# Equim-chan/Mortal

Hardware: NVIDIA H100
Metric: table-steps/sec batched self-play (higher is better)
Workload: dtype u8/i32 env + bf16 policy net

## Files before the change

include/mjx.h:

```cpp
#ifndef MJX_H
#define MJX_H
#include <stdint.h>

#ifdef __cplusplus
extern "C" {
#endif

enum mjx_status { MJX_OK = 0, MJX_ERR_CUDA = -1, MJX_ERR_ARG = -2, MJX_ERR_TABLES = -3, MJX_ERR_STATE = -4 };

#define MJX_ACTION_SPACE 46
#define MJX_OBS_COLS 34
#define MJX_MAX_ROWS_PER_TABLE 3

typedef struct mjx_env mjx_env;

const char* mjx_last_error(void);

int mjx_init(const char* data_dir, int device);

int mjx_obs_rows(int version);

int mjx_env_create(mjx_env** out, int n_tables, const uint64_t* nonces_host, const uint64_t* keys_host,
                   int obs_version, int shuffle_kind, int enable_quick_eval);
void mjx_env_destroy(mjx_env* env);
// ... 141 lines not shown
        forbidden_tiles[34], discarded_tiles[34];
    uint8_t akas_seen[3], akas_in_hand[3];
    uint8_t bakaze, jikaze, kyoku, honba, kyotaku, rank, oya, is_all_last;
    int32_t scores[4];
    uint8_t n_dora_indicators, dora_indicators[5];
    uint8_t riichi_declared[4], riichi_accepted[4];
    uint8_t at_turn, tiles_left;
    int8_t shanten, real_time_shanten;
    uint8_t has_last_self_tsumo, last_self_tsumo, has_last_kawa_tile, last_kawa_tile;
    uint32_t cans;
    uint8_t n_ankan_candidates, ankan_candidates[3], n_kakan_candidates, kakan_candidates[3];
    uint8_t chankan_chance, can_w_riichi, is_w_riichi, at_rinshan, at_ippatsu, at_furiten, to_mark_same_cycle_furiten,
        kans_on_board, is_menzen;
    uint8_t n_chis, chis[4], n_pons, pons[4], n_minkans, minkans[4], n_ankans, ankans[4];
    uint8_t doras_owned[4], doras_seen, tehai_len_div3, has_next_shanten_discard;
    uint8_t kawa_len[4];
    uint8_t viewer, pad_[3];
    int32_t err;
} mjx_player_view;
int mjx_state_create(mjx_env** out, int n, const uint8_t* player_ids_host, int obs_version);
int mjx_state_update(mjx_env* env, const uint64_t* words_host, const uint64_t* payload_host, uint32_t* cans_host);
int mjx_state_view(mjx_env* env, int index, mjx_player_view* out_host);
int mjx_state_rows(mjx_env* env, const uint8_t* at_kan_select_host, void* stream);
int mjx_state_query(mjx_env* env, int index, int what, const int32_t* args, int32_t* out);
int mjx_state_copy(mjx_env* dst, int dst_index, mjx_env* src, int src_index);

int mjx_env_set_encode_timing(mjx_env* env, int enable);
int mjx_env_last_encode_ms(mjx_env* env, float* ms_features, float* ms_store);

long long mjx_env_launch_count(mjx_env* env);

int mjx_env_row_cap(mjx_env* env);
uint8_t* mjx_env_masks(mjx_env* env);
int32_t* mjx_env_row_table(mjx_env* env);
uint8_t* mjx_env_row_seat(mjx_env* env);
uint32_t* mjx_env_row_step(mjx_env* env);
int32_t* mjx_env_num_rows_dev(mjx_env* env);

int mjx_env_results(mjx_env* env, void* stream, int32_t* scores_host , uint8_t* ranks_host ,
                    int32_t* steps_host , int32_t* err_host , int32_t* done_host );

int mjx_env_policy_test(mjx_env* env, int kind, int64_t* actions_dev, int64_t* trace_dev, float* q_values_dev,
                        void* stream);

int mjx_nn_affine_mish_bf16(const void* x, const float* scale, const float* bias, void* out, long long n_elems, int channels,
                            void* stream);
int mjx_nn_pool_bf16(const void* x, void* avg, void* mx, int batch, int length, int channels, void* stream);
int mjx_nn_gate_residual_bf16(const void* y, const void* gate, const void* x, void* out, int batch, int length, int channels,
                              void* stream);
int mjx_nn_obs_to_nhwc_bf16(const float* obs, void* out, int batch, int channels, int length, int channels_padded, void* stream);
int mjx_nn_block_tail_bf16(const void* y, const void* x, const float* w1, const float* b1, const float* w2t, const float* b2,
                           const float* scale, const float* bias, void* gate_scratch , void* x_out,
                           void* a_out, int batch, int length, int channels, int hidden, void* stream);

int mjx_shanten(const uint8_t* tiles_dev, const uint8_t* len_div3_dev, int8_t* out_dev, int n, void* stream);

typedef struct mjx_agari_in {
    uint8_t tehai[34];
    uint8_t chis[4], pons[4], minkans[4], ankans[4];
    uint8_t n_chis, n_pons, n_minkans, n_ankans;
    uint8_t bakaze, jikaze, winning_tile, is_ron;
    uint8_t additional_hans, doras;
    uint8_t is_oya, pad;
} mjx_agari_in;
typedef struct mjx_agari_out {
    uint8_t kind;
    uint8_t fu, han, yakuman;
    int32_t ron, tsumo_ko, tsumo_oya;
} mjx_agari_out;
int mjx_agari(const mjx_agari_in* in_dev, mjx_agari_out* out_dev, int n, int mode, void* stream);

int mjx_shanten_host(const uint8_t* tiles, const uint8_t* len_div3, int8_t* out, int n);
int mjx_agari_host(const mjx_agari_in* in, mjx_agari_out* out, int n, int mode);

int mjx_make_wall_host(uint64_t nonce, uint64_t key, int kyoku, int honba, int shuffle_kind, uint8_t* wall136);

#ifdef __cplusplus
}
#endif
#endif
```

mortal_b200/_lib.py:

```python
from __future__ import annotations

import ctypes as C
import os

HERE = os.path.dirname(os.path.abspath(__file__))
DATA_DIR = os.path.join(HERE, "data")
_LIB = None
_INIT_DEVICE = None


class MjxError(RuntimeError):
    pass


def lib_path() -> str:
    return os.path.join(HERE, "libmjx.so")


class AgariIn(C.Structure):
    _fields_ = [
        ("tehai", C.c_uint8 * 34),
        ("chis", C.c_uint8 * 4), ("pons", C.c_uint8 * 4), ("minkans", C.c_uint8 * 4), ("ankans", C.c_uint8 * 4),
        ("n_chis", C.c_uint8), ("n_pons", C.c_uint8), ("n_minkans", C.c_uint8), ("n_ankans", C.c_uint8),
        ("bakaze", C.c_uint8), ("jikaze", C.c_uint8), ("winning_tile", C.c_uint8), ("is_ron", C.c_uint8),
        ("additional_hans", C.c_uint8), ("doras", C.c_uint8), ("is_oya", C.c_uint8), ("pad", C.c_uint8),
    ]


class AgariOut(C.Structure):
    _fields_ = [("kind", C.c_uint8), ("fu", C.c_uint8), ("han", C.c_uint8), ("yakuman", C.c_uint8),
                ("ron", C.c_int32), ("tsumo_ko", C.c_int32), ("tsumo_oya", C.c_int32)]


SYMBOLS = {
    "mjx_last_error": (C.c_char_p, []),
    "mjx_init": (C.c_int, [C.c_char_p, C.c_int]),
    "mjx_obs_rows": (C.c_int, [C.c_int]),
    "mjx_env_create": (C.c_int, [C.POINTER(C.c_void_p), C.c_int, C.c_void_p, C.c_void_p, C.c_int, C.c_int, C.c_int]),
    "mjx_env_destroy": (None, [C.c_void_p]),
    "mjx_env_step": (C.c_int, [C.c_void_p, C.c_void_p, C.c_void_p, C.c_void_p]),
    "mjx_env_set_quick_eval": (C.c_int, [C.c_void_p, C.c_void_p]),
    "mjx_env_set_agari_guard": (C.c_int, [C.c_void_p, C.c_void_p]),
    "mjx_env_encode_obs": (C.c_int, [C.c_void_p, C.c_void_p, C.c_void_p]),
    "mjx_oracle_obs_rows": (C.c_int, [C.c_int]),
    "mjx_env_encode_invisible": (C.c_int, [C.c_void_p, C.c_void_p, C.c_int, C.c_void_p]),
    "mjx_env_set_obs_version": (C.c_int, [C.c_void_p, C.c_int]),
    "mjx_state_create": (C.c_int, [C.POINTER(C.c_void_p), C.c_int, C.c_void_p, C.c_int]),
    "mjx_state_update": (C.c_int, [C.c_void_p, C.c_void_p, C.c_void_p, C.c_void_p]),
    "mjx_state_view": (C.c_int, [C.c_void_p, C.c_int, C.c_void_p]),
    "mjx_state_rows": (C.c_int, [C.c_void_p, C.c_void_p, C.c_void_p]),
    "mjx_state_query": (C.c_int, [C.c_void_p, C.c_int, C.c_int, C.c_void_p, C.c_void_p]),
    "mjx_state_copy": (C.c_int, [C.c_void_p, C.c_int, C.c_void_p, C.c_int]),
    "mjx_env_set_sp": (C.c_int, [C.c_void_p, C.c_int]),
    "mjx_env_encode_obs_host": (C.c_int, [C.c_void_p, C.c_void_p, C.c_void_p, C.c_void_p, C.POINTER(C.c_int), C.c_void_p]),
    "mjx_env_encode_obs_host_begin": (C.c_int, [C.c_void_p, C.c_void_p, C.c_void_p, C.c_void_p, C.POINTER(C.c_int), C.c_void_p]),
    "mjx_env_encode_obs_host_finish": (C.c_int, [C.c_void_p]),
    "mjx_env_sp_overflows": (C.c_int, [C.c_void_p, C.c_void_p, C.POINTER(C.c_int)]),
    "mjx_env_sp_stats": (C.c_int, [C.c_void_p, C.c_void_p, C.POINTER(C.c_int)]),
    "mjx_env_enable_grp": (C.c_int, [C.c_void_p, C.c_int]),
    "mjx_env_read_grp": (C.c_int, [C.c_void_p, C.c_void_p, C.c_void_p, C.c_void_p]),
    "mjx_env_enable_log": (C.c_int, [C.c_void_p, C.c_int]),
    "mjx_env_log_len_dev": (C.c_void_p, [C.c_void_p]),
    "mjx_env_read_log": (C.c_int, [C.c_void_p, C.c_void_p, C.c_void_p, C.c_void_p]),
    "mjx_env_log_words_dev": (C.c_void_p, [C.c_void_p]),
    "mjx_meta_record_dev": (C.c_int, [C.c_longlong] + [C.c_void_p] * 4 + [C.c_int, C.c_int] + [C.c_void_p] * 5 + [C.c_int, C.c_int]
                            + [C.c_void_p] * 7 + [C.c_longlong, C.c_longlong, C.c_void_p]),
    "mjx_mjai_render_count_dev": (C.c_int, [C.c_int, C.c_void_p, C.c_void_p, C.c_int, C.c_void_p, C.c_int, C.c_int, C.c_void_p,
                                            C.c_void_p, C.c_void_p, C.c_void_p, C.c_void_p, C.c_longlong, C.c_void_p, C.c_void_p,
                                            C.c_void_p]),
    "mjx_mjai_render_fill_dev": (C.c_int, [C.c_int, C.c_void_p, C.c_void_p, C.c_int, C.c_void_p, C.c_int, C.c_int, C.c_void_p,
                                           C.c_void_p, C.c_void_p, C.c_void_p, C.c_void_p, C.c_longlong, C.c_void_p, C.c_void_p,
                                           C.c_int, C.c_int, C.c_void_p, C.c_longlong, C.c_void_p]),
    "mjx_nn_affine_mish_bf16": (C.c_int, [C.c_void_p, C.c_void_p, C.c_void_p, C.c_void_p, C.c_longlong, C.c_int, C.c_void_p]),
    "mjx_nn_pool_bf16": (C.c_int, [C.c_void_p, C.c_void_p, C.c_void_p, C.c_int, C.c_int, C.c_int, C.c_void_p]),
    "mjx_nn_gate_residual_bf16": (C.c_int, [C.c_void_p, C.c_void_p, C.c_void_p, C.c_void_p, C.c_int, C.c_int, C.c_int, C.c_void_p]),
    "mjx_nn_obs_to_nhwc_bf16": (C.c_int, [C.c_void_p, C.c_void_p, C.c_int, C.c_int, C.c_int, C.c_int, C.c_void_p]),
    "mjx_nn_block_tail_bf16": (C.c_int, [C.c_void_p] * 11 + [C.c_int, C.c_int, C.c_int, C.c_int, C.c_void_p]),
    "mjx_env_create_replay": (C.c_int, [C.POINTER(C.c_void_p), C.c_int, C.c_void_p, C.c_void_p, C.c_void_p, C.c_longlong, C.c_void_p,
                                        C.c_void_p, C.c_longlong, C.c_void_p, C.c_int, C.c_int]),
    "mjx_env_create_replay_dev": (C.c_int, [C.POINTER(C.c_void_p), C.c_int, C.c_void_p, C.c_void_p, C.c_void_p, C.c_longlong,
                                            C.c_void_p, C.c_void_p, C.c_longlong, C.c_void_p, C.c_int, C.c_int, C.c_void_p]),
    "mjx_env_replay_trust_seeds": (C.c_int, [C.c_void_p, C.c_void_p, C.c_void_p, C.c_int]),
    "mjx_env_replay_step": (C.c_int, [C.c_void_p, C.c_void_p]),
    "mjx_env_replay_viewpoints": (C.c_int, [C.c_void_p, C.c_void_p]),
    "mjx_env_row_label": (C.c_void_p, [C.c_void_p]),
    "mjx_env_row_meta": (C.c_void_p, [C.c_void_p]),
    "mjx_env_set_encode_timing": (C.c_int, [C.c_void_p, C.c_int]),
    "mjx_env_last_encode_ms": (C.c_int, [C.c_void_p, C.POINTER(C.c_float), C.POINTER(C.c_float)]),
    "mjx_env_launch_count": (C.c_longlong, [C.c_void_p]),
    "mjx_env_num_rows": (C.c_int, [C.c_void_p, C.c_void_p, C.POINTER(C.c_int)]),
    "mjx_env_poll": (C.c_int, [C.c_void_p, C.c_void_p, C.POINTER(C.c_int)]),
    "mjx_env_num_live": (C.c_int, [C.c_void_p, C.c_void_p, C.POINTER(C.c_int)]),
    "mjx_env_total_steps": (C.c_int, [C.c_void_p, C.c_void_p, C.POINTER(C.c_int64)]),
    "mjx_env_row_cap": (C.c_int, [C.c_void_p]),
    "mjx_env_masks": (C.c_void_p, [C.c_void_p]),
    "mjx_env_row_table": (C.c_void_p, [C.c_void_p]),
    "mjx_env_row_seat": (C.c_void_p, [C.c_void_p]),
    "mjx_env_row_step": (C.c_void_p, [C.c_void_p]),
    "mjx_env_num_rows_dev": (C.c_void_p, [C.c_void_p]),
    "mjx_env_results": (C.c_int, [C.c_void_p, C.c_void_p, C.c_void_p, C.c_void_p, C.c_void_p, C.c_void_p, C.c_void_p]),
    "mjx_env_policy_test": (C.c_int, [C.c_void_p, C.c_int, C.c_void_p, C.c_void_p, C.c_void_p, C.c_void_p]),
    "mjx_shanten": (C.c_int, [C.c_void_p, C.c_void_p, C.c_void_p, C.c_int, C.c_void_p]),
    "mjx_agari": (C.c_int, [C.c_void_p, C.c_void_p, C.c_int, C.c_int, C.c_void_p]),
    "mjx_shanten_host": (C.c_int, [C.c_void_p, C.c_void_p, C.c_void_p, C.c_int]),
    "mjx_agari_host": (C.c_int, [C.c_void_p, C.c_void_p, C.c_int, C.c_int]),
    "mjx_make_wall_host": (C.c_int, [C.c_uint64, C.c_uint64, C.c_int, C.c_int, C.c_int, C.c_void_p]),
    "mjx_validate_logs": (C.c_int, [C.c_int, C.c_void_p, C.c_void_p, C.c_void_p, C.c_longlong, C.c_void_p, C.c_void_p, C.c_longlong,
                                    C.c_void_p, C.c_void_p, C.c_longlong, C.c_void_p, C.c_void_p]),
    "mjx_validate_logs_dev": (C.c_int, [C.c_int, C.c_void_p, C.c_void_p, C.c_void_p, C.c_longlong, C.c_void_p, C.c_void_p,
                                        C.c_longlong, C.c_void_p, C.c_void_p, C.c_longlong, C.c_void_p, C.c_void_p]),
    "mjx_mjai_count_dev": (C.c_int, [C.c_int, C.c_void_p, C.c_longlong, C.c_void_p, C.c_int, C.c_void_p, C.c_void_p]),
    "mjx_mjai_fill_dev": (C.c_int, [C.c_int, C.c_void_p, C.c_longlong, C.c_void_p, C.c_int, C.c_void_p, C.c_void_p, C.c_void_p,
                                    C.c_void_p, C.c_void_p, C.c_void_p, C.c_longlong, C.c_void_p, C.c_longlong, C.c_void_p,
                                    C.c_longlong, C.c_void_p]),
    "mjx_mjai_fill_deltas_dev": (C.c_int, [C.c_int, C.c_void_p, C.c_longlong, C.c_void_p, C.c_int, C.c_void_p, C.c_void_p,
                                           C.c_void_p, C.c_void_p, C.c_void_p, C.c_void_p, C.c_longlong, C.c_void_p, C.c_longlong,
                                           C.c_void_p, C.c_longlong, C.c_void_p, C.c_void_p, C.c_void_p]),
    "mjx_stat_logs_dev": (C.c_int, [C.c_int, C.c_void_p, C.c_void_p, C.c_void_p, C.c_longlong, C.c_void_p, C.c_void_p, C.c_longlong,
                                    C.c_void_p, C.c_void_p, C.c_void_p, C.c_void_p, C.c_void_p, C.c_void_p]),
    "mjx_grp_logs_dev": (C.c_int, [C.c_int, C.c_void_p, C.c_void_p, C.c_void_p, C.c_longlong, C.c_void_p, C.c_void_p, C.c_longlong,
                                   C.c_void_p, C.c_void_p, C.c_void_p, C.c_void_p, C.c_void_p, C.c_void_p, C.c_void_p]),
}


def load():
    global _LIB
    if _LIB is not None:
        return _LIB
    path = lib_path()
    if not os.path.exists(path):
# ... 25 lines not shown
```

mortal_b200/csrc/mjx_kernels.cu:

```cuda
#include <cstdio>
#include <cstring>
#include <mutex>
#include <string>
#include <vector>

#include "../../include/mjx.h"
#include "mjx_sp.cuh"
#include "mjx_policy.cuh"
#include "mjx_replay.cuh"
#include "mjx_validate.cuh"
#include "mjx_mjai.cuh"
#include "mjx_mjai_write.cuh"
#include "mjx_stat.cuh"
#include "mjx_grp.cuh"
#include "mjx_invisible.cuh"
#include "mjx_state.cuh"
#include "mjx_nn.cuh"
#include "mjx_tables_host.h"

using namespace mjx;

constexpr int STEP_WARPS = 4;

__global__ void __launch_bounds__(STEP_WARPS * 32) k_step(EnvView V, Tables T) {
    __shared__ __align__(16) unsigned char s_tab[STEP_WARPS][sizeof(TableState)];
    __shared__ WarpScratch s_scratch[STEP_WARPS];
    const int warp = threadIdx.x >> 5, lane = threadIdx.x & 31;
    const int table = blockIdx.x * STEP_WARPS + warp;
    if (table >= V.n_tables) return;
    TableState* g = V.tables + table;
    if (!(g->gflags & GF_ALIVE)) return;
    constexpr int NV = sizeof(TableState) / 16;
    uint4* dst = reinterpret_cast<uint4*>(s_tab[warp]);
    const uint4* src = reinterpret_cast<const uint4*>(g);
    for (int i = lane; i < NV; i += 32) dst[i] = src[i];
    __syncwarp();
    Ctx c;
    c.S = reinterpret_cast<TableState*>(s_tab[warp]);
    c.W = &s_scratch[warp];
    c.T = T;
    c.lane = lane;
    c.df = s_scratch[warp].dora_factor;
    if (V.log) { c.log = V.log + (size_t)table * V.log_cap; c.log_n = V.log_len + table; c.log_cap = V.log_cap; }
    if (V.grp) { c.grp = V.grp + (size_t)table * V.grp_cap * 7; c.grp_n = V.grp_len + table; c.grp_cap = V.grp_cap; }
    const i32 err_before = c.S->err;
    const bool live = step_table(c, V, table);
    __syncwarp();
    uint4* gdst = reinterpret_cast<uint4*>(g);
    for (int i = lane; i < NV; i += 32) gdst[i] = dst[i];
    if (lane == 0 && live) {
        atomicAdd(&V.counters[0], 1ull);
        atomicAdd(&V.counters[1], 1ull);
    }
    if (lane == 0 && err_before == 0 && c.S->err != 0) atomicAdd(&V.counters[2], 1ull);
}

__global__ void __launch_bounds__(STEP_WARPS * 32) k_replay_step(EnvView V, ReplayView R, Tables T) {
    __shared__ __align__(16) unsigned char s_tab[STEP_WARPS][sizeof(TableState)];
    __shared__ WarpScratch s_scratch[STEP_WARPS];
    const int warp = threadIdx.x >> 5, lane = threadIdx.x & 31;
    const int job = blockIdx.x * STEP_WARPS + warp;
    if (job >= V.n_tables) return;
    TableState* g = V.tables + job;
    if (!(g->gflags & GF_ALIVE)) return;
    constexpr int NV = sizeof(TableState) / 16;
    uint4* dst = reinterpret_cast<uint4*>(s_tab[warp]);
    const uint4* src = reinterpret_cast<const uint4*>(g);
    for (int i = lane; i < NV; i += 32) dst[i] = src[i];
    __syncwarp();
    Ctx c;
// ... 1741 lines not shown
int mjx_nn_affine_mish_bf16(const void* x, const float* scale, const float* bias, void* out, long long n_elems, int channels,
                            void* stream) {
    if (!x || !scale || !bias || !out || channels <= 0 || channels % 8 || n_elems % channels)
        return fail(MJX_ERR_ARG, "mjx_nn_affine_mish_bf16: bad arguments");
    if (!g_ready) return fail(MJX_ERR_STATE, "mjx_nn_*: call mjx_init first");
    const size_t n_vec = (size_t)n_elems / 8;
    mjx_nn::k_affine_mish<<<nn_grid_for(n_vec, channels / 8), 256, 0, (cudaStream_t)stream>>>((const mjx_nn::Vec8*)x, scale, bias, (mjx_nn::Vec8*)out,
                                                                            n_vec, channels / 8);
    CU(cudaGetLastError());
    return MJX_OK;
}
int mjx_nn_pool_bf16(const void* x, void* avg, void* mx, int batch, int length, int channels, void* stream) {
    if (!x || !avg || !mx || batch <= 0 || length <= 0 || channels <= 0 || channels % 8)
        return fail(MJX_ERR_ARG, "mjx_nn_pool_bf16: bad arguments");
    if (!g_ready) return fail(MJX_ERR_STATE, "mjx_nn_*: call mjx_init first");
    mjx_nn::k_pool<<<nn_grid((size_t)batch * (channels / 8)), 256, 0, (cudaStream_t)stream>>>(
        (const mjx_nn::Vec8*)x, (mjx_nn::Vec8*)avg, (mjx_nn::Vec8*)mx, batch, length, channels / 8);
    CU(cudaGetLastError());
    return MJX_OK;
}
int mjx_nn_obs_to_nhwc_bf16(const float* obs, void* out, int batch, int channels, int length, int channels_padded, void* stream) {
    if (!obs || !out || batch <= 0 || channels <= 0 || length <= 0 || length > 128 || channels_padded < channels ||
        channels_padded % mjx_nn::NHWC_TC)
        return fail(MJX_ERR_ARG, "mjx_nn_obs_to_nhwc_bf16: bad arguments (channels_padded a multiple of 64, length <= 128)");
    if (!g_ready) return fail(MJX_ERR_STATE, "mjx_nn_*: call mjx_init first");
    const size_t smem = (size_t)mjx_nn::NHWC_TC * (length + 1) * sizeof(float);
    const long long grid = (long long)batch * (channels_padded / mjx_nn::NHWC_TC);
    if (grid > 0x7fffffffLL) return fail(MJX_ERR_ARG, "mjx_nn_obs_to_nhwc_bf16: batch too large");
    mjx_nn::k_obs_to_nhwc<<<(int)grid, 256, smem, (cudaStream_t)stream>>>(obs, (__nv_bfloat16*)out, channels, length, channels_padded);
    CU(cudaGetLastError());
    return MJX_OK;
}
int mjx_nn_block_tail_bf16(const void* y, const void* x, const float* w1, const float* b1, const float* w2t, const float* b2,
                           const float* scale, const float* bias, void* gate_scratch, void* x_out, void* a_out, int batch, int length,
                           int channels, int hidden, void* stream) {
    if (!y || !x || !w1 || !b1 || !w2t || !b2 || !scale || !bias || !gate_scratch || !x_out || !a_out || batch <= 0 || length <= 0 ||
        channels <= 0 || channels % 8 || channels > 256 || hidden <= 0 || hidden > 64)
        return fail(MJX_ERR_ARG, "mjx_nn_block_tail_bf16: bad arguments (channels % 8 == 0, <= 256; hidden <= 64)");
    if (!g_ready) return fail(MJX_ERR_STATE, "mjx_nn_*: call mjx_init first");
    cudaStream_t st = (cudaStream_t)stream;
    const int c8 = channels / 8;
    const int warps_per_cta = 8;
    const int grid = std::max(1, std::min((batch + warps_per_cta - 1) / warps_per_cta, g_sm_count * 8));
    mjx_nn::k_pool_gate<<<grid, warps_per_cta * 32, 0, st>>>((const mjx_nn::Vec8*)y, w1, b1, w2t, b2, (mjx_nn::Vec8*)gate_scratch, batch, length,
                                                               c8, hidden);
    CU(cudaGetLastError());
    const size_t n_vec = (size_t)batch * length * c8;
    mjx_nn::k_gate_residual_mish<<<nn_grid_for(n_vec, c8), 256, 0, st>>>(
        (const mjx_nn::Vec8*)y, (const mjx_nn::Vec8*)gate_scratch, (const mjx_nn::Vec8*)x, scale, bias, (mjx_nn::Vec8*)x_out,
        (mjx_nn::Vec8*)a_out, n_vec, length, c8);
    CU(cudaGetLastError());
    return MJX_OK;
}
int mjx_nn_gate_residual_bf16(const void* y, const void* gate, const void* x, void* out, int batch, int length, int channels,
                              void* stream) {
    if (!y || !gate || !x || !out || batch <= 0 || length <= 0 || channels <= 0 || channels % 8)
        return fail(MJX_ERR_ARG, "mjx_nn_gate_residual_bf16: bad arguments");
    if (!g_ready) return fail(MJX_ERR_STATE, "mjx_nn_*: call mjx_init first");
    const size_t n_vec = (size_t)batch * length * (channels / 8);
    mjx_nn::k_gate_residual<<<nn_grid(n_vec), 256, 0, (cudaStream_t)stream>>>((const mjx_nn::Vec8*)y, (const mjx_nn::Vec8*)gate,
                                                                              (const mjx_nn::Vec8*)x, (mjx_nn::Vec8*)out, n_vec,
                                                                              length, channels / 8);
    CU(cudaGetLastError());
    return MJX_OK;
}

int mjx_shanten(const uint8_t* tiles_dev, const uint8_t* len_dev, int8_t* out_dev, int n, void* stream) {
    if (!g_ready) return fail(MJX_ERR_STATE, "mjx_shanten: call mjx_init first");
    if (n <= 0) return MJX_OK;
    k_shanten<<<(n + SH_THREADS - 1) / SH_THREADS, SH_THREADS, 0, (cudaStream_t)stream>>>(g_T, tiles_dev, len_dev,
                                                                                         (i8*)out_dev, n);
    CU(cudaGetLastError());
    return MJX_OK;
}

int mjx_agari(const mjx_agari_in* in_dev, mjx_agari_out* out_dev, int n, int mode, void* stream) {
    if (!g_ready) return fail(MJX_ERR_STATE, "mjx_agari: call mjx_init first");
    if (mode < 0 || mode > 3) return fail(MJX_ERR_ARG, "mjx_agari: mode must be 0..3");
    if (n <= 0) return MJX_OK;
    k_agari<<<(n + 127) / 128, 128, 0, (cudaStream_t)stream>>>(g_T, in_dev, out_dev, n, mode);
    CU(cudaGetLastError());
    return MJX_OK;
}

namespace {
struct HostScratch {
    std::mutex mu;
    void* p[3] = {nullptr, nullptr, nullptr};
    size_t cap[3] = {0, 0, 0};
    int reserve(int i, size_t bytes, void** out) {
        if (cap[i] < bytes) {
            cudaFree(p[i]); p[i] = nullptr; cap[i] = 0;
            size_t want = 1 << 16;
            while (want < bytes) want <<= 1;
            cudaError_t e = cudaMalloc(&p[i], want);
            if (e != cudaSuccess) return fail(MJX_ERR_CUDA, cudaGetErrorString(e));
            cap[i] = want;
        }
        *out = p[i];
        return MJX_OK;
    }
};
HostScratch g_host_scratch;
}

int mjx_shanten_host(const uint8_t* tiles, const uint8_t* len_div3, int8_t* out, int n) {
// ... 48 lines not shown
```

mortal_b200/model.py:

```python
from __future__ import annotations

import torch
from torch import nn

OBS_ROWS = {1: 938, 2: 942, 3: 934, 4: 1012}
ACTION_SPACE = 46


class ChannelGate(nn.Module):
    def __init__(self, channels: int, ratio: int = 16):
        super().__init__()
        self.fc1 = nn.Linear(channels, channels // ratio)
        self.fc2 = nn.Linear(channels // ratio, channels)
        nn.init.zeros_(self.fc1.bias)
        nn.init.zeros_(self.fc2.bias)
        self.act = nn.Mish(inplace=True)

    def _mlp(self, v):
        return self.fc2(self.act(self.fc1(v)))

    def forward(self, x):
        gate = torch.sigmoid(self._mlp(x.mean(-1)) + self._mlp(x.amax(-1)))
        return x * gate.unsqueeze(-1)

# ... 24 lines not shown
        return scale.view(1, -1, 1, 1).contiguous(), shift.view(1, -1, 1, 1).contiguous()

    def forward_fast(self, x, aff, w1, w2, aff32=None):
        (s1, b1), (s2, b2) = aff
        F = torch.nn.functional
        if aff32 is not None and x.is_cuda and x.dtype == torch.bfloat16:
            from . import nn_ops

            (f1, g1), (f2, g2) = aff32
            y = F.conv2d(nn_ops.affine_mish(x, f1, g1), w1, padding=(0, 1))
            y = F.conv2d(nn_ops.affine_mish(y, f2, g2), w2, padding=(0, 1))
            avg, mx = nn_ops.pool_mean_max(y)
            h = self.gate._mlp(torch.cat((avg, mx), 0))
            gate = torch.sigmoid(h[: avg.shape[0]] + h[avg.shape[0]:])
            return nn_ops.gate_residual(y, gate.contiguous(), x)
        y = F.conv2d(F.mish(torch.addcmul(b1, x, s1)), w1, padding=(0, 1))
        y = F.conv2d(F.mish(torch.addcmul(b2, y, s2)), w2, padding=(0, 1))
        return self.gate.forward_fast(y) + x


class Brain(nn.Module):
    def __init__(self, *, conv_channels: int = 192, num_blocks: int = 40, version: int = 4):
        super().__init__()
        assert version == 4, "only the version-4 network is restated here"
        self.version = version
        c = conv_channels
        self.stem = nn.Conv1d(OBS_ROWS[version], c, 3, padding=1, bias=False)
        self.blocks = nn.Sequential(*[PreActBlock(c) for _ in range(num_blocks)])
        self.bn = nn.BatchNorm1d(c, momentum=0.01, eps=1e-3)
        self.act = nn.Mish(inplace=True)
        self.neck = nn.Conv1d(c, 32, 3, padding=1)
        self.fc = nn.Linear(32 * 34, 1024)

    def forward(self, obs):
        x = self.blocks(self.stem(obs))
        x = self.act(self.neck(self.act(self.bn(x))))
        return self.act(self.fc(x.flatten(1)))

    @torch.no_grad()
    def prepare_fast(self, dtype=None):
        assert not self.training, "prepare_fast() is for eval mode"
        flat = lambda a: (a[0].float().flatten().contiguous(), a[1].float().flatten().contiguous())
        self._aff32 = [(flat(PreActBlock._affine(b.bn1)), flat(PreActBlock._affine(b.bn2))) for b in self.blocks]
        self._aff32_out = flat(PreActBlock._affine(self.bn))
        if dtype is not None:
            self.to(dtype)
        self._aff = [(PreActBlock._affine(b.bn1), PreActBlock._affine(b.bn2)) for b in self.blocks]
        self._aff_out = PreActBlock._affine(self.bn)
        f32 = lambda t: t.detach().float().contiguous()
        self._gate32 = [(f32(b.gate.fc1.weight), f32(b.gate.fc1.bias), f32(b.gate.fc2.weight.t()), f32(b.gate.fc2.bias)) for b in self.blocks]
        cl = lambda conv: conv.weight.unsqueeze(2).contiguous(memory_format=torch.channels_last)
        self._w = [(cl(b.conv1), cl(b.conv2)) for b in self.blocks]
        self._w_stem, self._w_neck = cl(self.stem), cl(self.neck)
        cin = self.stem.weight.shape[1]
        self._cpad = (cin + 63) // 64 * 64
        wp = torch.zeros((self.stem.weight.shape[0], self._cpad, 3), dtype=self.stem.weight.dtype, device=self.stem.weight.device)
        wp[:, :cin] = self.stem.weight.detach()
        self._w_stem_pad = wp.unsqueeze(2).contiguous(memory_format=torch.channels_last)
        self._fast_dtype = dtype
        return self

    def forward_fast(self, obs):
        F = torch.nn.functional
        fused = obs.is_cuda and self._fast_dtype == torch.bfloat16
        if fused and obs.dtype == torch.float32 and obs.is_contiguous():
            from . import nn_ops

            x = F.conv2d(nn_ops.obs_to_nhwc(obs, self._cpad), self._w_stem_pad, padding=(0, 1))
        else:
            if self._fast_dtype is not None:
                obs = obs.to(self._fast_dtype)
            x = obs.unsqueeze(2).contiguous(memory_format=torch.channels_last)
            x = F.conv2d(x, self._w_stem, padding=(0, 1))
        if fused:
            from . import nn_ops

            n = len(self.blocks)
            a = nn_ops.affine_mish(x, *self._aff32[0][0]) if n else nn_ops.affine_mish(x, *self._aff32_out)
            for i in range(n):
                (w1, w2), (_, (f2, g2)) = self._w[i], self._aff32[i]
                y = F.conv2d(a, w1, padding=(0, 1))
                y = F.conv2d(nn_ops.affine_mish(y, f2, g2), w2, padding=(0, 1))
                nxt = self._aff32[i + 1][0] if i + 1 < n else self._aff32_out
                x, a = nn_ops.block_tail(y, x, *self._gate32[i], *nxt)
            x = a
        else:
            for blk, aff, (w1, w2) in zip(self.blocks, self._aff, self._w):
                x = blk.forward_fast(x, aff, w1, w2, None)
            s, b = self._aff_out
            x = F.mish(torch.addcmul(b, x, s))
        x = F.mish(F.conv2d(x, self._w_neck, self.neck.bias, padding=(0, 1)))
        return F.mish(self.fc(x.flatten(1)))


class DQN(nn.Module):
    def __init__(self, *, version: int = 4):
        super().__init__()
        assert version == 4
        self.net = nn.Linear(1024, 1 + ACTION_SPACE)
        nn.init.zeros_(self.net.bias)

    def forward(self, phi, mask):
        v, a = self.net(phi).split((1, ACTION_SPACE), dim=-1)
        a_mean = a.masked_fill(~mask, 0.0).sum(-1, keepdim=True) / mask.sum(-1, keepdim=True)
        return (v + a - a_mean).masked_fill(~mask, -torch.inf)
```

mortal_b200/nn_ops.py:

```python
from __future__ import annotations

import ctypes as C

import torch

from . import _lib


def _stream(t: torch.Tensor):
    return C.c_void_p(torch.cuda.current_stream(t.device).cuda_stream)


def _check_nhwc(x: torch.Tensor):
    assert x.is_cuda and x.dtype == torch.bfloat16 and x.dim() == 4 and x.shape[2] == 1
    b, c, _, l = x.shape
    assert c % 8 == 0 and x.stride(1) == 1 and x.stride(3) == c and x.stride(0) == c * l, "expected channels_last [B, C, 1, L]"
    return b, c, l


def affine_mish(x: torch.Tensor, scale: torch.Tensor, bias: torch.Tensor) -> torch.Tensor:
    b, c, l = _check_nhwc(x)
    assert scale.dtype == torch.float32 and bias.dtype == torch.float32 and scale.numel() == c == bias.numel()
    out = torch.empty_like(x)
    _lib.check(_lib.load().mjx_nn_affine_mish_bf16(C.c_void_p(x.data_ptr()), C.c_void_p(scale.data_ptr()), C.c_void_p(bias.data_ptr()),
                                                   C.c_void_p(out.data_ptr()), x.numel(), c, _stream(x)), "mjx_nn_affine_mish_bf16")
    return out


def pool_mean_max(x: torch.Tensor):
    b, c, l = _check_nhwc(x)
    avg = torch.empty((b, c), dtype=torch.bfloat16, device=x.device)
    mx = torch.empty((b, c), dtype=torch.bfloat16, device=x.device)
    _lib.check(_lib.load().mjx_nn_pool_bf16(C.c_void_p(x.data_ptr()), C.c_void_p(avg.data_ptr()), C.c_void_p(mx.data_ptr()), b, l, c,
                                            _stream(x)), "mjx_nn_pool_bf16")
    return avg, mx


def gate_residual(y: torch.Tensor, gate: torch.Tensor, x: torch.Tensor) -> torch.Tensor:
    b, c, l = _check_nhwc(y)
    assert _check_nhwc(x) == (b, c, l) and gate.dtype == torch.bfloat16 and gate.shape == (b, c) and gate.is_contiguous()
    out = torch.empty_like(y)
    _lib.check(_lib.load().mjx_nn_gate_residual_bf16(C.c_void_p(y.data_ptr()), C.c_void_p(gate.data_ptr()), C.c_void_p(x.data_ptr()),
                                                     C.c_void_p(out.data_ptr()), b, l, c, _stream(y)), "mjx_nn_gate_residual_bf16")
    return out


def block_tail(y: torch.Tensor, x: torch.Tensor, w1: torch.Tensor, b1: torch.Tensor, w2t: torch.Tensor, b2: torch.Tensor,
               scale: torch.Tensor, bias: torch.Tensor):
    b, c, l = _check_nhwc(y)
    assert _check_nhwc(x) == (b, c, l)
    h = w1.shape[0]
    for t, shape in ((w1, (h, c)), (b1, (h,)), (w2t, (h, c)), (b2, (c,)), (scale, (c,)), (bias, (c,))):
        assert t.dtype == torch.float32 and tuple(t.shape) == shape and t.is_contiguous() and t.is_cuda
    assert c <= 256, "block_tail: at most 256 channels"
    x_out, a_out = torch.empty_like(y), torch.empty_like(y)
    gate = torch.empty((b, c), dtype=torch.bfloat16, device=y.device)
    p = lambda t: C.c_void_p(t.data_ptr())
    _lib.check(_lib.load().mjx_nn_block_tail_bf16(p(y), p(x), p(w1), p(b1), p(w2t), p(b2), p(scale), p(bias), p(gate), p(x_out), p(a_out),
                                                  b, l, c, h, _stream(y)), "mjx_nn_block_tail_bf16")
    return x_out, a_out


def obs_to_nhwc(obs: torch.Tensor, channels_padded: int) -> torch.Tensor:
    assert obs.is_cuda and obs.dtype == torch.float32 and obs.dim() == 3 and obs.is_contiguous()
    b, c, l = obs.shape
    assert channels_padded >= c and channels_padded % 64 == 0
    out = torch.empty((b, channels_padded, 1, l), dtype=torch.bfloat16, device=obs.device, memory_format=torch.channels_last)
    _lib.check(_lib.load().mjx_nn_obs_to_nhwc_bf16(C.c_void_p(obs.data_ptr()), C.c_void_p(out.data_ptr()), b, c, l, channels_padded,
                                                   _stream(obs)), "mjx_nn_obs_to_nhwc_bf16")
    return out
```

Baseline: 245,800.

## Add warp-specialized TMA+WGMMA conv3 kernel with fused affine-mish epilogue for residual blocks

Replaces the cuDNN F.conv2d calls in each residual block with a custom Hopper kernel. It uses TMA bulk loads into an 8-stage mbarrier pipeline, a producer warpgroup, and consumer warpgroups issuing m64n192k16 WGMMA as an implicit GEMM over three taps, with boundary rows zeroed in shared memory. The first conv fuses the affine+mish epilogue, which removes a separate elementwise kernel and its memory round trip. The kernel is hardcoded to 192 channels and length 34, and the zeroing of padded rows plus the swizzle descriptors carry correctness risk.

```diff
diff --git a/include/mjx.h b/include/mjx.h
--- a/include/mjx.h
+++ b/include/mjx.h
@@ -217,6 +217,8 @@
 int mjx_nn_block_tail_bf16(const void* y, const void* x, const float* w1, const float* b1, const float* w2t, const float* b2,
                            const float* scale, const float* bias, void* gate_scratch , void* x_out,
                            void* a_out, int batch, int length, int channels, int hidden, void* stream);
+int mjx_nn_conv3_bf16(const void* x, const void* w, const float* scale, const float* bias, void* out, int batch, int length, int channels,
+                      int epilogue, void* stream);
 
 int mjx_shanten(const uint8_t* tiles_dev, const uint8_t* len_div3_dev, int8_t* out_dev, int n, void* stream);
 
diff --git a/mortal_b200/_lib.py b/mortal_b200/_lib.py
--- a/mortal_b200/_lib.py
+++ b/mortal_b200/_lib.py
@@ -76,6 +76,7 @@
     "mjx_nn_gate_residual_bf16": (C.c_int, [C.c_void_p, C.c_void_p, C.c_void_p, C.c_void_p, C.c_int, C.c_int, C.c_int, C.c_void_p]),
     "mjx_nn_obs_to_nhwc_bf16": (C.c_int, [C.c_void_p, C.c_void_p, C.c_int, C.c_int, C.c_int, C.c_int, C.c_void_p]),
     "mjx_nn_block_tail_bf16": (C.c_int, [C.c_void_p] * 11 + [C.c_int, C.c_int, C.c_int, C.c_int, C.c_void_p]),
+    "mjx_nn_conv3_bf16": (C.c_int, [C.c_void_p] * 5 + [C.c_int, C.c_int, C.c_int, C.c_int, C.c_void_p]),
     "mjx_env_create_replay": (C.c_int, [C.POINTER(C.c_void_p), C.c_int, C.c_void_p, C.c_void_p, C.c_void_p, C.c_longlong, C.c_void_p,
                                         C.c_void_p, C.c_longlong, C.c_void_p, C.c_int, C.c_int]),
     "mjx_env_create_replay_dev": (C.c_int, [C.POINTER(C.c_void_p), C.c_int, C.c_void_p, C.c_void_p, C.c_void_p, C.c_longlong,
diff --git a/mortal_b200/csrc/mjx_conv.cuh b/mortal_b200/csrc/mjx_conv.cuh
--- /dev/null
+++ b/mortal_b200/csrc/mjx_conv.cuh
@@ -0,0 +1,173 @@
+#pragma once
+#include <cuda.h>
+#include <cuda_bf16.h>
+#include <cuda_runtime.h>
+#include <stdint.h>
+
+#include "mjx_nn.cuh"
+
+namespace mjx_nn {
+
+constexpr int CV_C = 192, CV_L = 34;
+constexpr int CV_BM = 192, CV_BK = 32;
+constexpr int CV_KSTEPS = 3 * (CV_C / CV_BK);
+constexpr int CV_STAGES = 8;
+constexpr int CV_CONSUMERS = CV_BM / 64;
+constexpr int CV_THREADS = (CV_CONSUMERS + 1) * 128;
+constexpr int CV_A_BYTES = CV_BM * CV_BK * 2, CV_B_BYTES = CV_C * CV_BK * 2;
+constexpr int CV_OUT_BYTES = 64 * 64 * 2;
+constexpr int CV_SMEM = CV_STAGES * (CV_A_BYTES + CV_B_BYTES) + CV_CONSUMERS * CV_OUT_BYTES + 2 * CV_STAGES * 8 + 1024;
+enum { CV_EPI_PLAIN = 0, CV_EPI_AFFINE_MISH = 1 };
+
+__device__ __forceinline__ uint32_t cv_smem(const void* p) { return (uint32_t)__cvta_generic_to_shared(p); }
+__device__ __forceinline__ void cv_bar_init(uint32_t bar, uint32_t count) {
+    asm volatile("mbarrier.init.shared::cta.b64 [%0], %1;" ::"r"(bar), "r"(count) : "memory");
+}
+__device__ __forceinline__ void cv_bar_expect_tx(uint32_t bar, uint32_t bytes) {
+    asm volatile("mbarrier.arrive.expect_tx.shared::cta.b64 _, [%0], %1;" ::"r"(bar), "r"(bytes) : "memory");
+}
+__device__ __forceinline__ void cv_bar_arrive(uint32_t bar) {
+    asm volatile("mbarrier.arrive.shared::cta.b64 _, [%0];" ::"r"(bar) : "memory");
+}
+__device__ __forceinline__ void cv_bar_wait(uint32_t bar, uint32_t parity) {
+    uint32_t done;
+    do {
+        asm volatile("{ .reg .pred p; mbarrier.try_wait.parity.shared::cta.b64 p, [%1], %2; selp.u32 %0, 1, 0, p; }"
+                     : "=r"(done) : "r"(bar), "r"(parity) : "memory");
+    } while (!done);
+}
+__device__ __forceinline__ void cv_tma_load(uint32_t dst, const CUtensorMap* map, int c0, int c1, uint32_t bar) {
+    asm volatile("cp.async.bulk.tensor.2d.shared::cluster.global.mbarrier::complete_tx::bytes [%0], [%1, {%2, %3}], [%4];"
+                 ::"r"(dst), "l"(reinterpret_cast<uint64_t>(map)), "r"(c0), "r"(c1), "r"(bar) : "memory");
+}
+__device__ __forceinline__ void cv_tma_store(const CUtensorMap* map, int c0, int c1, uint32_t src) {
+    asm volatile("cp.async.bulk.tensor.2d.global.shared::cta.bulk_group [%0, {%1, %2}], [%3];"
+                 ::"l"(reinterpret_cast<uint64_t>(map)), "r"(c0), "r"(c1), "r"(src) : "memory");
+}
+__device__ __forceinline__ void cv_fence_async_smem() { asm volatile("fence.proxy.async.shared::cta;" ::: "memory"); }
+__device__ __forceinline__ void cv_wg_sync(int wg) {
+    asm volatile("bar.sync %0, 128;" ::"r"(wg + 1) : "memory");
+}
+
+__device__ __forceinline__ uint64_t cv_desc(uint32_t saddr) {
+    return (uint64_t)((saddr & 0x3FFFF) >> 4) | (uint64_t)1 << 16 | (uint64_t)(512 >> 4) << 32 | (uint64_t)2 << 62;
+}
+
+#define CV_D8(i) "+f"(d[i + 0]), "+f"(d[i + 1]), "+f"(d[i + 2]), "+f"(d[i + 3]), "+f"(d[i + 4]), "+f"(d[i + 5]), "+f"(d[i + 6]), "+f"(d[i + 7])
+__device__ __forceinline__ void cv_wgmma(float* d, uint64_t da, uint64_t db, int scale_d) {
+    asm volatile(
+        "{ .reg .pred p; setp.ne.b32 p, %98, 0;\n"
+        "wgmma.mma_async.sync.aligned.m64n192k16.f32.bf16.bf16 "
+        "{%0, %1, %2, %3, %4, %5, %6, %7, %8, %9, %10, %11, %12, %13, %14, %15, %16, %17, %18, %19, %20, %21, %22, %23, "
+        "%24, %25, %26, %27, %28, %29, %30, %31, %32, %33, %34, %35, %36, %37, %38, %39, %40, %41, %42, %43, %44, %45, %46, %47, "
+        "%48, %49, %50, %51, %52, %53, %54, %55, %56, %57, %58, %59, %60, %61, %62, %63, %64, %65, %66, %67, %68, %69, %70, %71, "
+        "%72, %73, %74, %75, %76, %77, %78, %79, %80, %81, %82, %83, %84, %85, %86, %87, %88, %89, %90, %91, %92, %93, %94, %95}, "
+        "%96, %97, p, 1, 1, 0, 0; }\n"
+        : CV_D8(0), CV_D8(8), CV_D8(16), CV_D8(24), CV_D8(32), CV_D8(40), CV_D8(48), CV_D8(56), CV_D8(64), CV_D8(72), CV_D8(80), CV_D8(88)
+        : "l"(da), "l"(db), "r"(scale_d));
+}
+#undef CV_D8
+
+template <int EPI>
+__global__ void __launch_bounds__(CV_THREADS, 1) k_conv3_wgmma(const __grid_constant__ CUtensorMap map_a, const __grid_constant__ CUtensorMap map_w,
+                                                               const __grid_constant__ CUtensorMap map_out, const float* __restrict__ scale,
+                                                               const float* __restrict__ bias, int m_rows) {
+    extern __shared__ uint8_t cv_raw[];
+    const uint32_t base = (cv_smem(cv_raw) + 1023) & ~1023u;
+    uint8_t* const gbase = cv_raw + (base - cv_smem(cv_raw));
+    const uint32_t sa = base, sb = sa + CV_STAGES * CV_A_BYTES, so = sb + CV_STAGES * CV_B_BYTES;
+    const uint32_t full = so + CV_CONSUMERS * CV_OUT_BYTES, empty = full + CV_STAGES * 8;
+    const int n_tiles = (m_rows + CV_BM - 1) / CV_BM;
+    const int tid = threadIdx.x, wg = tid >> 7;
+
+    if (tid == 0) {
+        for (int s = 0; s < CV_STAGES; s++) {
+            cv_bar_init(full + 8 * s, 1);
+            cv_bar_init(empty + 8 * s, CV_CONSUMERS);
+        }
+        asm volatile("fence.mbarrier_init.release.cluster;" ::: "memory");
+        cv_fence_async_smem();
+    }
+    __syncthreads();
+
+    if (wg == CV_CONSUMERS) {
+        asm volatile("setmaxnreg.dec.sync.aligned.u32 40;");
+        if (tid == CV_CONSUMERS * 128) {
+            int it = 0;
+            for (int tile = blockIdx.x; tile < n_tiles; tile += gridDim.x) {
+                for (int ks = 0; ks < CV_KSTEPS; ks++, it++) {
+                    const int s = it % CV_STAGES, tap = ks % 3, c0 = (ks / 3) * CV_BK;
+                    cv_bar_wait(empty + 8 * s, ((it / CV_STAGES) & 1) ^ 1);
+                    cv_bar_expect_tx(full + 8 * s, CV_A_BYTES + CV_B_BYTES);
+                    cv_tma_load(sa + s * CV_A_BYTES, &map_a, c0, tile * CV_BM + tap - 1, full + 8 * s);
+                    cv_tma_load(sb + s * CV_B_BYTES, &map_w, c0, tap * CV_C, full + 8 * s);
+                }
+            }
+        }
+        return;
+    }
+
+    asm volatile("setmaxnreg.inc.sync.aligned.u32 152;");
+    const int t = tid & 127, warp = t >> 5, lane = t & 31;
+    const uint32_t stage_out = so + wg * CV_OUT_BYTES;
+    float d[96];
+    int it = 0;
+    for (int tile = blockIdx.x; tile < n_tiles; tile += gridDim.x) {
+        const int m0 = tile * CV_BM + 64 * wg;
+        for (int ks = 0; ks < CV_KSTEPS; ks++, it++) {
+            const int s = it % CV_STAGES, tap = ks % 3;
+            cv_bar_wait(full + 8 * s, (it / CV_STAGES) & 1);
+            const uint32_t a_s = sa + s * CV_A_BYTES + wg * 64 * (CV_BK * 2);
+            if (tap != 1) {
+                const int r = t >> 1;
+                if ((m0 + r) % CV_L == (tap == 0 ? 0 : CV_L - 1)) {
+                    uint4* p = reinterpret_cast<uint4*>(gbase + (a_s - base) + r * (CV_BK * 2) + (t & 1) * CV_BK);
+                    p[0] = make_uint4(0u, 0u, 0u, 0u);
+                    p[1] = make_uint4(0u, 0u, 0u, 0u);
+                }
+                cv_fence_async_smem();
+                cv_wg_sync(wg);
+            }
+            asm volatile("wgmma.fence.sync.aligned;" ::: "memory");
+            const uint64_t da = cv_desc(a_s), db = cv_desc(sb + s * CV_B_BYTES);
+#pragma unroll
+            for (int kk = 0; kk < CV_BK / 16; kk++) cv_wgmma(d, da + 2 * kk, db + 2 * kk, ks > 0 || kk > 0);
+            asm volatile("wgmma.commit_group.sync.aligned;" ::: "memory");
+            asm volatile("wgmma.wait_group.sync.aligned 1;" ::: "memory");
+            if (ks > 0 && t == 0) cv_bar_arrive(empty + 8 * ((it - 1) % CV_STAGES));
+        }
+        asm volatile("wgmma.wait_group.sync.aligned 0;" ::: "memory");
+        if (t == 0) cv_bar_arrive(empty + 8 * ((it - 1) % CV_STAGES));
+
+        const int r0 = 16 * warp + (lane >> 2);
+#pragma unroll
+        for (int b = 0; b < CV_C / 64; b++) {
+            if (t == 0) asm volatile("cp.async.bulk.wait_group.read 0;" ::: "memory");
+            cv_wg_sync(wg);
+#pragma unroll
+            for (int j = 8 * b; j < 8 * b + 8; j++) {
+                const int n = 8 * j + 2 * (lane & 3);
+                float v0 = d[4 * j], v1 = d[4 * j + 1], v2 = d[4 * j + 2], v3 = d[4 * j + 3];
+                if (EPI == CV_EPI_AFFINE_MISH) {
+                    const float2 sc = __ldg(reinterpret_cast<const float2*>(scale + n)), bi = __ldg(reinterpret_cast<const float2*>(bias + n));
+                    v0 = mish_f(fmaf(bf16_round(v0), sc.x, bi.x)); v1 = mish_f(fmaf(bf16_round(v1), sc.y, bi.y));
+                    v2 = mish_f(fmaf(bf16_round(v2), sc.x, bi.x)); v3 = mish_f(fmaf(bf16_round(v3), sc.y, bi.y));
+                }
+                const __nv_bfloat162 h0 = __floats2bfloat162_rn(v0, v1), h1 = __floats2bfloat162_rn(v2, v3);
+                const uint32_t p0 = stage_out + r0 * 128 + (((j & 7) ^ (r0 & 7)) << 4) + 4 * (lane & 3);
+                const uint32_t p1 = stage_out + (r0 + 8) * 128 + (((j & 7) ^ ((r0 + 8) & 7)) << 4) + 4 * (lane & 3);
+                asm volatile("st.shared.b32 [%0], %1;" ::"r"(p0), "r"(*reinterpret_cast<const uint32_t*>(&h0)) : "memory");
+                asm volatile("st.shared.b32 [%0], %1;" ::"r"(p1), "r"(*reinterpret_cast<const uint32_t*>(&h1)) : "memory");
+            }
+            cv_fence_async_smem();
+            cv_wg_sync(wg);
+            if (t == 0 && m0 < m_rows) {
+                cv_tma_store(&map_out, 64 * b, m0, stage_out);
+                asm volatile("cp.async.bulk.commit_group;" ::: "memory");
+            }
+        }
+    }
+    if (t == 0) asm volatile("cp.async.bulk.wait_group 0;" ::: "memory");
+}
+
+}
diff --git a/mortal_b200/csrc/mjx_kernels.cu b/mortal_b200/csrc/mjx_kernels.cu
--- a/mortal_b200/csrc/mjx_kernels.cu
+++ b/mortal_b200/csrc/mjx_kernels.cu
@@ -16,6 +16,7 @@
 #include "mjx_invisible.cuh"
 #include "mjx_state.cuh"
 #include "mjx_nn.cuh"
+#include "mjx_conv.cuh"
 #include "mjx_tables_host.h"
 
 using namespace mjx;
@@ -1863,6 +1864,58 @@
     CU(cudaGetLastError());
     return MJX_OK;
 }
+typedef CUresult (*cv_encode_fn)(CUtensorMap*, CUtensorMapDataType, cuuint32_t, void*, const cuuint64_t*, const cuuint64_t*,
+                                 const cuuint32_t*, const cuuint32_t*, CUtensorMapInterleave, CUtensorMapSwizzle,
+                                 CUtensorMapL2promotion, CUtensorMapFloatOOBfill);
+static int cv_tensor_map(CUtensorMap* map, const void* ptr, long long rows, int cols, int box_rows, int box_cols) {
+    static cv_encode_fn encode = nullptr;
+    if (!encode) {
+        void* fn = nullptr;
+        cudaDriverEntryPointQueryResult q;
+        CU(cudaGetDriverEntryPointByVersion("cuTensorMapEncodeTiled", &fn, 12000, cudaEnableDefault, &q));
+        if (q != cudaDriverEntryPointSuccess || !fn) return fail(MJX_ERR_CUDA, "cuTensorMapEncodeTiled: entry point not found");
+        encode = (cv_encode_fn)fn;
+    }
+    const cuuint64_t dims[2] = {(cuuint64_t)cols, (cuuint64_t)rows}, strides[1] = {(cuuint64_t)cols * 2};
+    const cuuint32_t box[2] = {(cuuint32_t)box_cols, (cuuint32_t)box_rows}, elem[2] = {1, 1};
+    const CUresult r = encode(map, CU_TENSOR_MAP_DATA_TYPE_BFLOAT16, 2, const_cast<void*>(ptr), dims, strides, box, elem,
+                              CU_TENSOR_MAP_INTERLEAVE_NONE, box_cols == 64 ? CU_TENSOR_MAP_SWIZZLE_128B : CU_TENSOR_MAP_SWIZZLE_64B,
+                              CU_TENSOR_MAP_L2_PROMOTION_L2_256B,
+                              CU_TENSOR_MAP_FLOAT_OOB_FILL_NONE);
+    if (r != CUDA_SUCCESS) return fail(MJX_ERR_CUDA, "cuTensorMapEncodeTiled failed: " + std::to_string((int)r));
+    return MJX_OK;
+}
+static int cv_launch(bool affine, const CUtensorMap& a, const CUtensorMap& w, const CUtensorMap& o, const float* scale, const float* bias,
+                     int m_rows, cudaStream_t st) {
+    static bool attr[2] = {false, false};
+    const auto kernel = affine ? mjx_nn::k_conv3_wgmma<mjx_nn::CV_EPI_AFFINE_MISH> : mjx_nn::k_conv3_wgmma<mjx_nn::CV_EPI_PLAIN>;
+    if (!attr[affine]) {
+        CU(cudaFuncSetAttribute(kernel, cudaFuncAttributeMaxDynamicSharedMemorySize, mjx_nn::CV_SMEM));
+        attr[affine] = true;
+    }
+    const int tiles = (m_rows + mjx_nn::CV_BM - 1) / mjx_nn::CV_BM;
+    kernel<<<std::min(tiles, g_sm_count), mjx_nn::CV_THREADS, mjx_nn::CV_SMEM, st>>>(a, w, o, scale, bias, m_rows);
+    CU(cudaGetLastError());
+    return MJX_OK;
+}
+int mjx_nn_conv3_bf16(const void* x, const void* w, const float* scale, const float* bias, void* out, int batch, int length, int channels,
+                      int epilogue, void* stream) {
+    const bool affine = epilogue == mjx_nn::CV_EPI_AFFINE_MISH;
+    if (!x || !w || !out || batch <= 0 || (epilogue != mjx_nn::CV_EPI_PLAIN && !affine) || (affine && (!scale || !bias)) ||
+        ((uintptr_t)x | (uintptr_t)w | (uintptr_t)out) % 16 || (affine && ((uintptr_t)scale | (uintptr_t)bias) % 8))
+        return fail(MJX_ERR_ARG, "mjx_nn_conv3_bf16: bad arguments");
+    if (channels != mjx_nn::CV_C || length != mjx_nn::CV_L)
+        return fail(MJX_ERR_ARG, "mjx_nn_conv3_bf16: only channels == 192 and length == 34");
+    const long long m_rows = (long long)batch * length;
+    if (m_rows > 0x7fffffffLL - mjx_nn::CV_BM) return fail(MJX_ERR_ARG, "mjx_nn_conv3_bf16: batch too large");
+    if (!g_ready) return fail(MJX_ERR_STATE, "mjx_nn_*: call mjx_init first");
+    CUtensorMap ma, mw, mo;
+    int rc;
+    if ((rc = cv_tensor_map(&ma, x, m_rows, channels, mjx_nn::CV_BM, mjx_nn::CV_BK)) ||
+        (rc = cv_tensor_map(&mw, w, 3LL * channels, channels, channels, mjx_nn::CV_BK)) || (rc = cv_tensor_map(&mo, out, m_rows, channels, 64, 64)))
+        return rc;
+    return cv_launch(affine, ma, mw, mo, scale, bias, (int)m_rows, (cudaStream_t)stream);
+}
 int mjx_nn_gate_residual_bf16(const void* y, const void* gate, const void* x, void* out, int batch, int length, int channels,
                               void* stream) {
     if (!y || !gate || !x || !out || batch <= 0 || length <= 0 || channels <= 0 || channels % 8)
diff --git a/mortal_b200/model.py b/mortal_b200/model.py
--- a/mortal_b200/model.py
+++ b/mortal_b200/model.py
@@ -100,6 +100,11 @@
         cl = lambda conv: conv.weight.unsqueeze(2).contiguous(memory_format=torch.channels_last)
         self._w = [(cl(b.conv1), cl(b.conv2)) for b in self.blocks]
         self._w_stem, self._w_neck = cl(self.stem), cl(self.neck)
+        self._w3 = None
+        if dtype == torch.bfloat16 and self.stem.weight.shape[0] == 192:
+            from . import nn_ops
+
+            self._w3 = [(nn_ops.conv3_weight(b.conv1.weight), nn_ops.conv3_weight(b.conv2.weight)) for b in self.blocks]
         cin = self.stem.weight.shape[1]
         self._cpad = (cin + 63) // 64 * 64
         wp = torch.zeros((self.stem.weight.shape[0], self._cpad, 3), dtype=self.stem.weight.dtype, device=self.stem.weight.device)
@@ -126,9 +131,14 @@
             n = len(self.blocks)
             a = nn_ops.affine_mish(x, *self._aff32[0][0]) if n else nn_ops.affine_mish(x, *self._aff32_out)
             for i in range(n):
-                (w1, w2), (_, (f2, g2)) = self._w[i], self._aff32[i]
-                y = F.conv2d(a, w1, padding=(0, 1))
-                y = F.conv2d(nn_ops.affine_mish(y, f2, g2), w2, padding=(0, 1))
+                (_, (f2, g2)) = self._aff32[i]
+                if self._w3 is not None:
+                    w1, w2 = self._w3[i]
+                    y = nn_ops.conv3(nn_ops.conv3(a, w1, f2, g2), w2)
+                else:
+                    w1, w2 = self._w[i]
+                    y = F.conv2d(a, w1, padding=(0, 1))
+                    y = F.conv2d(nn_ops.affine_mish(y, f2, g2), w2, padding=(0, 1))
                 nxt = self._aff32[i + 1][0] if i + 1 < n else self._aff32_out
                 x, a = nn_ops.block_tail(y, x, *self._gate32[i], *nxt)
             x = a
diff --git a/mortal_b200/nn_ops.py b/mortal_b200/nn_ops.py
--- a/mortal_b200/nn_ops.py
+++ b/mortal_b200/nn_ops.py
@@ -61,6 +61,22 @@
     return x_out, a_out
 
 
+def conv3(x: torch.Tensor, w: torch.Tensor, scale: torch.Tensor | None = None, bias: torch.Tensor | None = None) -> torch.Tensor:
+    b, c, l = _check_nhwc(x)
+    assert w.is_cuda and w.dtype == torch.bfloat16 and tuple(w.shape) == (3, c, c) and w.is_contiguous()
+    affine = scale is not None
+    if affine:
+        assert scale.dtype == torch.float32 and bias.dtype == torch.float32 and scale.numel() == c == bias.numel()
+    out = torch.empty_like(x)
+    p = lambda t: C.c_void_p(t.data_ptr() if t is not None else 0)
+    _lib.check(_lib.load().mjx_nn_conv3_bf16(p(x), p(w), p(scale), p(bias), p(out), b, l, c, int(affine), _stream(x)), "mjx_nn_conv3_bf16")
+    return out
+
+
+def conv3_weight(w: torch.Tensor) -> torch.Tensor:
+    return w.detach().permute(2, 0, 1).to(torch.bfloat16).contiguous()
+
+
 def obs_to_nhwc(obs: torch.Tensor, channels_padded: int) -> torch.Tensor:
     assert obs.is_cuda and obs.dtype == torch.float32 and obs.dim() == 3 and obs.is_contiguous()
     b, c, l = obs.shape
```

Result: faster. 252,400 (median of 6 runs) (+2.7%).
